# chengruiz/cusrl

Hardware: AMD Instinct MI355X
Metric: env_steps_per_sec (higher is better)
Workload: dtype f32; 1 GPU; synthetic continuous env 4096x obs48 x act12 per GPU, MLP(256,128) actor-critic, rollout_len=24, ppo preset (5 epochs x 4 minibatches, Adam lr 2e-4); envs_per_gpu=4096, parallelism=dp1, rccl_ranks=0, collectives=none (single process), hipgraph=True, fused_env=True, captured_env_steps=24, epoch_graph_updates=432, unjoined_steps_captured=20, autoreset=False

## Files before the change

__graft_entry__.py:

```python

from __future__ import annotations

import os
import subprocess
import sys
from pathlib import Path

ROOT = Path(__file__).resolve().parent
CSRC = ROOT / "cusrl_amd" / "csrc"
LIB = ROOT / "cusrl_amd" / "libcusrl_hip.so"
HIP_SOURCES = ["api.hip", "buffer.hip", "advantage.hip", "ppo_loss.hip", "rollout.hip", "policy_stats.hip", "policy_terms.hip", "mlp_epilogue.hip", "input_layer.hip", "mlp_forward.hip", "gradient.hip", "narrow_linear.hip", "normalization.hip", "recurrent.hip", "aux_hooks.hip", "gru.hip", "comm.hip", "symmetry.hip", "smoothness.hip", "layer_norm.hip", "column_affine.hip", "gate.hip", "attention.hip", "conv.hip", "bijector.hip", "bias_act.hip", "deploy.hip", "environment.hip", "reward_norm.hip", "frame_stack.hip"]
HIPCC_FLAGS = [
    "--offload-arch=gfx950",
    "-O3",
    "-std=c++17",
    "-ffp-contract=off",
    "-fPIC",
    "-shared",
    "-ldl",
]


def _stale(target: Path, sources: list[Path]) -> bool:
    return not target.exists() or any(src.stat().st_mtime > target.stat().st_mtime for src in sources)


def build(force: bool = False) -> None:
    from concurrent.futures import ThreadPoolExecutor

    sources = [CSRC / name for name in HIP_SOURCES]
    headers = [*sorted(CSRC.glob("*.hpp")), ROOT / "include" / "cusrl_hip.h"]
    hipcc = os.environ.get("HIPCC", "/opt/rocm/bin/hipcc")
    objdir = ROOT / "build" / "obj"
    objdir.mkdir(parents=True, exist_ok=True)
    compile_flags = [f for f in HIPCC_FLAGS if f not in ("-shared", "-ldl")]

    def compile_one(src: Path) -> Path:
        obj = objdir / (src.stem + ".o")
        if force or _stale(obj, [src, *headers]):
            subprocess.run([hipcc, *compile_flags, f"-I{ROOT / 'include'}", f"-I{CSRC}", "-c", str(src), "-o", str(obj)], check=True)
        return obj

    with ThreadPoolExecutor(max_workers=min(8, os.cpu_count() or 1)) as pool:
        objects = list(pool.map(compile_one, sources))
    if force or _stale(LIB, objects):
        subprocess.run([hipcc, "--offload-arch=gfx950", "-shared", "-fPIC", "-s", *map(str, objects), "-ldl", "-o", str(LIB)], check=True)
    if str(ROOT) not in sys.path:
        sys.path.insert(0, str(ROOT))
    import oracle

    oracle.build(force=force)
    import cusrl_amd
    from cusrl_amd import _native

    _native.lib()
    assert cusrl_amd.__name__ == "cusrl_amd"


def smoke() -> None:
    if str(ROOT) not in sys.path:
        sys.path.insert(0, str(ROOT))
    import numpy as np
    import torch

    import cusrl_amd as cusrl
    import oracle

    assert torch.cuda.is_available(), "smoke() needs an MI355X"
    cusrl.config.set_device("cuda:0")
    cusrl.set_global_seed(0)
    env = cusrl.testing.SyntheticEnvironment(num_instances=256, observation_dim=48, action_dim=12, device="cuda:0")
    factory = cusrl.preset.PpoAgentFactory(num_steps_per_update=8, sampler_epochs=2, sampler_mini_batches=2)
    trainer = cusrl.Trainer(env, factory, num_iterations=2, verbose=False)
    trainer.run_training_loop()
    buffer = trainer.agent.buffer
    host = {k: buffer[k].cpu().numpy() for k in ("reward", "value", "next_value", "done", "advantage", "return")}
    adv, ret = oracle.gae(host["reward"], host["done"], host["value"], host["next_value"], 0.99, 0.95)
    assert np.array_equal(ret, host["return"]), "return differs from the oracle"
    var, mean = oracle.var_mean(adv)
    np.testing.assert_allclose(oracle.normalize(adv, mean, var), host["advantage"], rtol=1e-5, atol=1e-5)
    torch.cuda.synchronize()
    print("smoke ok: 2 iterations of the ppo preset on cuda:0, GAE/return bit-exact vs oracle")


if __name__ == "__main__":
    build(force="--force" in sys.argv)
    print(f"built {LIB}")
```

cusrl_amd/csrc/narrow_linear.hip:

```cpp
#include <stdlib.h>

#include "common.hpp"

namespace cusrl {

static int head_rows_per_block() {
    const int v = int(option(kOptHeadRows));
    return v >= 8 && v <= 4096 ? v : 96;
}
constexpr int head_batch(int O) { return O > 8 ? 2 : 4; }
constexpr int kHeadBiasPad = 16;

template <int O, bool kReluInput>
__global__ __launch_bounds__(kBlock) void narrow_linear_bwd_kernel(const float *__restrict__ grad_out,
                                                                   const float *__restrict__ input,
                                                                   const float *__restrict__ weight,
                                                                   float *__restrict__ grad_input,
                                                                   float *__restrict__ partials, int64_t rows, int K,
                                                                   int rows_per_block) {
    extern __shared__ float4 red[];
    constexpr int SL = O + 1;
    const int lpr = K / 4;
    const int groups = kBlock / lpr;
    const int col = threadIdx.x % lpr, sub = threadIdx.x / lpr;
// ... 95 lines not shown
            total.x += (a.x + b.x) + (c.x + d.x), total.y += (a.y + b.y) + (c.y + d.y);
            total.z += (a.z + b.z) + (c.z + d.z), total.w += (a.w + b.w) + (c.w + d.w);
        }
        for (; p < P; p += 16) {
            const float4 a = base[p * stride];
            total.x += a.x, total.y += a.y, total.z += a.z, total.w += a.w;
        }
    }
    red[threadIdx.x] = total;
    __syncthreads();
    if (group == 0 && h < H) {
        float4 sum = red[c4];
        for (int g = 1; g < 16; ++g) {
            const float4 v = red[g * 16 + c4];
            sum.x += v.x, sum.y += v.y, sum.z += v.z, sum.w += v.w;
        }
        *reinterpret_cast<float4 *>(out + h) = sum;
    }
}


template <int kLanes>
__global__ __launch_bounds__(kBlock) void narrow_dot_fwd_kernel(const float *__restrict__ input, const float *__restrict__ weight,
                                                                const float *__restrict__ bias, float *__restrict__ output,
                                                                int64_t rows, int K) {
    constexpr int kRowsPerWave = kWave / kLanes, kInFlight = 4;
    const int lane = threadIdx.x & (kWave - 1);
    const int sub = lane % kLanes, rloc = lane / kLanes;
    const int chunks = K / 4;
    const int64_t wave = int64_t(blockIdx.x) * kWavesPerBlock + threadIdx.x / kWave;
    const int64_t row0 = wave * (kRowsPerWave * kInFlight);
    if (row0 >= rows) return;
    const float b = bias ? bias[0] : 0.f;
    float acc[kInFlight] = {0.f, 0.f, 0.f, 0.f};
    for (int c = sub; c < chunks; c += kLanes) {
        const float4 w = reinterpret_cast<const float4 *>(weight)[c];
        float4 x[kInFlight];
#pragma unroll
        for (int k = 0; k < kInFlight; ++k) {
            const int64_t row = min(row0 + int64_t(k) * kRowsPerWave + rloc, rows - 1);
            x[k] = reinterpret_cast<const float4 *>(input)[row * chunks + c];
        }
#pragma unroll
        for (int k = 0; k < kInFlight; ++k)
            acc[k] += (x[k].x * w.x + x[k].y * w.y) + (x[k].z * w.z + x[k].w * w.w);
    }
#pragma unroll
    for (int k = 0; k < kInFlight; ++k) {
        float v = acc[k];
#pragma unroll
        for (int off = kLanes / 2; off > 0; off >>= 1) v += __shfl_xor(v, off, kWave);
        const int64_t row = row0 + int64_t(k) * kRowsPerWave + rloc;
        if (sub == 0 && row < rows) output[row] = v + b;
    }
}

static bool narrow_shape_ok(int64_t K, int64_t O) {
    if (O < 1 || O > 16 || K < 32 || K > 1024 || K % 4) return false;
    const int64_t lpr = K / 4;
    return (lpr & (lpr - 1)) == 0;
}

template <int O, bool kReluInput>
static int launch_narrow_bwd_as(const float *grad_out, const float *input, const float *weight, float *grad_input,
                                float *partials, int64_t rows, int K, int64_t blocks, hipStream_t s) {
    const int lpr = K / 4, groups = kBlock / lpr;
    const size_t lds = size_t(groups) * (O + 1) * lpr * sizeof(float4) + size_t(groups) * kHeadBiasPad * sizeof(float);
    if (lds > 64 * 1024) {
        hipError_t err = hipFuncSetAttribute(reinterpret_cast<const void *>(&narrow_linear_bwd_kernel<O, kReluInput>),
                                             hipFuncAttributeMaxDynamicSharedMemorySize, int(lds));
        if (err != hipSuccess) return int(err);
    }
    hipLaunchKernelGGL((narrow_linear_bwd_kernel<O, kReluInput>), dim3(uint32_t(blocks)), dim3(kBlock), lds, s, grad_out,
                       input, weight, grad_input, partials, rows, K, head_rows_per_block());
    return launch_status();
}

template <int O>
static int launch_narrow_bwd(const float *grad_out, const float *input, const float *weight, float *grad_input,
                             float *partials, int64_t rows, int K, int64_t blocks, bool relu_input, hipStream_t s) {
    return relu_input ? launch_narrow_bwd_as<O, true>(grad_out, input, weight, grad_input, partials, rows, K, blocks, s)
                      : launch_narrow_bwd_as<O, false>(grad_out, input, weight, grad_input, partials, rows, K, blocks, s);
}

}

extern "C" int cusrl_narrow_linear_supported(int64_t in_features, int64_t out_features) {
    return cusrl::narrow_shape_ok(in_features, out_features) ? 1 : 0;
}

extern "C" int64_t cusrl_narrow_linear_num_partials(int64_t rows) {
    return rows <= 0 ? 0 : cusrl::ceil_div(rows, int64_t(cusrl::head_rows_per_block()));
}

extern "C" int cusrl_narrow_linear_bwd(const float *grad_out, const float *input, const float *weight,
                                       float *grad_input, float *partials, float *packed, int64_t rows,
                                       int64_t in_features, int64_t out_features, int relu_input, void *stream) {
    using namespace cusrl;
    if (!grad_out || !input || !weight || !partials || rows <= 0) return CUSRL_E_INVALID;
    if (!narrow_shape_ok(in_features, out_features)) return CUSRL_E_UNSUPPORTED;
    if (out_features % 4 == 0 && !aligned(grad_out, 16)) return CUSRL_E_UNSUPPORTED;
    if (!aligned(input, 16) || !aligned(weight, 16) || !aligned(partials, 16) || (packed && !aligned(packed, 16)) ||
        (grad_input && !aligned(grad_input, 16)))
        return CUSRL_E_UNSUPPORTED;
    hipStream_t s = as_stream(stream);
    const int K = int(in_features);
    const int64_t blocks = ceil_div(rows, int64_t(head_rows_per_block()));
    const bool relu = relu_input != 0;
    int rc = 0;
    switch (out_features) {
#define CUSRL_NARROW_CASE(N) \
    case N: rc = launch_narrow_bwd<N>(grad_out, input, weight, grad_input, partials, rows, K, blocks, relu, s); break;
        CUSRL_NARROW_CASE(1) CUSRL_NARROW_CASE(2) CUSRL_NARROW_CASE(3) CUSRL_NARROW_CASE(4)
        CUSRL_NARROW_CASE(5) CUSRL_NARROW_CASE(6) CUSRL_NARROW_CASE(7) CUSRL_NARROW_CASE(8)
        CUSRL_NARROW_CASE(9) CUSRL_NARROW_CASE(10) CUSRL_NARROW_CASE(11) CUSRL_NARROW_CASE(12)
        CUSRL_NARROW_CASE(13) CUSRL_NARROW_CASE(14) CUSRL_NARROW_CASE(15) CUSRL_NARROW_CASE(16)
#undef CUSRL_NARROW_CASE
        default: return CUSRL_E_UNSUPPORTED;
    }
    if (rc) return rc;
    if (!packed) return 0;
    const int H = (int(out_features) + 1) * K + kHeadBiasPad;
    hipLaunchKernelGGL(narrow_linear_finalize_kernel, dim3(uint32_t(ceil_div(H, 64))), dim3(kBlock), 0, s, partials,
                       blocks, H, packed);
    return launch_status();
}

extern "C" int cusrl_narrow_linear_fwd(const float *input, const float *weight, const float *bias, float *output,
                                       int64_t rows, int64_t in_features, int64_t out_features, void *stream) {
    using namespace cusrl;
    if (!input || !weight || !output || rows <= 0) return CUSRL_E_INVALID;
    if (out_features != 1 || !narrow_shape_ok(in_features, 1)) return CUSRL_E_UNSUPPORTED;
    if (!aligned(input, 16) || !aligned(weight, 16)) return CUSRL_E_UNSUPPORTED;
    const int K = int(in_features), lanes = K / 4 >= kWave ? kWave : K / 4;
    const int64_t waves = ceil_div(rows, int64_t(kWave / lanes) * 4), blocks = ceil_div(waves, int64_t(kWavesPerBlock));
    if (blocks > INT32_MAX) return CUSRL_E_UNSUPPORTED;
    hipStream_t s = as_stream(stream);
    switch (lanes) {
#define CUSRL_DOT_CASE(N)                                                                                              \
    case N:                                                                                                            \
        hipLaunchKernelGGL(narrow_dot_fwd_kernel<N>, dim3(uint32_t(blocks)), dim3(kBlock), 0, s, input, weight, bias,   \
                           output, rows, K);                                                                           \
        break;
        CUSRL_DOT_CASE(8) CUSRL_DOT_CASE(16) CUSRL_DOT_CASE(32) CUSRL_DOT_CASE(64)
#undef CUSRL_DOT_CASE
        default: return CUSRL_E_UNSUPPORTED;
    }
    return launch_status();
}
```

cusrl_amd/nn/module.py:

```python

from __future__ import annotations

from collections.abc import Iterable, Sequence
from contextlib import contextmanager
from dataclasses import dataclass
from typing import Any

import torch
from torch import nn
from torch.nn.functional import linear

from cusrl_amd.utils import switches
from cusrl_amd.utils.nest import iterate_nested

__all__ = ["Linear", "LinearFp32", "fused_inference_layers", "linear_act", "Mlp", "Module", "ModuleFactory", "disable_autocast",
           "double_differentiable", "is_unit_gradient", "register_unit_gradient", "resolve_activation_fn", "saved_gradients"]


def disable_autocast(device_type: str):
    return torch.autocast(device_type=device_type, enabled=False)


_split_grad_sink: dict[int, torch.Tensor] | None = None


_plain_linear_depth = 0
_WIDE_MIN_ROWS = switches.read("WIDE_LINEAR_MIN_ROWS")
_INPUT_LAYER_KERNEL = switches.read("INPUT_LAYER_KERNEL")


_unit_gradients: dict[int, "weakref.ref[torch.Tensor]"] = {}


def register_unit_gradient(ones: torch.Tensor) -> torch.Tensor:
    import weakref

    address = ones.data_ptr()
    _unit_gradients[address] = weakref.ref(ones)
    weakref.finalize(ones, _forget_unit_gradient, address)
    return ones


def _forget_unit_gradient(address: int) -> None:
    ref = _unit_gradients.get(address)
    if ref is not None and ref() is None:
        del _unit_gradients[address]


def is_unit_gradient(grad: torch.Tensor | None) -> bool:
    if grad is None or grad.dim() != 0:
        return False
    ref = _unit_gradients.get(grad.data_ptr())
    return ref is not None and ref() is not None


def saved_gradients(gradients, grad_loss) -> list:
    if is_unit_gradient(grad_loss):
        return list(gradients)
    return [gradient * grad_loss for gradient in gradients]


@contextmanager
def double_differentiable():
    global _plain_linear_depth
    _plain_linear_depth += 1
    try:
        yield
    finally:
        _plain_linear_depth -= 1


@contextmanager
def collect_split_weight_grads():
    global _split_grad_sink
    previous, _split_grad_sink = _split_grad_sink, {}
    try:
        yield _split_grad_sink
    finally:
        _split_grad_sink = previous


def _hand_over(sink, key, gradient):
    from cusrl_amd import ops

    if not isinstance(gradient, ops.DeferredColumns):
        return gradient
    if sink is not None and key is not None and key not in sink:
        sink[key] = gradient
        return None
    return gradient.materialize()


class _WideBatchLinear(torch.autograd.Function):

    @staticmethod
    def forward(ctx, input, weight, bias, splits, relu):
        if relu:
            output = torch._addmm_activation(bias, input, weight.t())
            ctx.save_for_backward(input, weight, output)
            output._cusrl_relu_output = True
        else:
            output = _one_output_linear(input, weight, bias)
            ctx.save_for_backward(input, weight)
        ctx.splits, ctx.relu, ctx.has_bias = splits, relu, bias is not None
        ctx.bias_key = bias.data_ptr() if bias is not None else None
        ctx.narrow = ((not relu) and input.is_contiguous() and weight.is_contiguous() and input.data_ptr() % 16 == 0
                      and _narrow_head(weight))
        ctx.input_is_relu_output = getattr(input, "_cusrl_relu_output", False)
        return output

    @staticmethod
    @torch.autograd.function.once_differentiable
    def backward(ctx, grad_output):
        from cusrl_amd import ops

        if ctx.relu:
            input, weight, output = ctx.saved_tensors
            sink = _split_grad_sink
            premasked = getattr(grad_output, "_cusrl_premasked", None)
            if (_INPUT_LAYER_KERNEL and premasked is None and not ctx.needs_input_grad[0] and ctx.needs_input_grad[1]
                    and ctx.has_bias and ctx.needs_input_grad[2]):
                grad_output = grad_output.contiguous()
                if ops.input_layer_supported(grad_output, output, input, weight):
                    d_weight, d_bias = ops.input_layer_backward(grad_output, output, input)
                    return None, d_weight, d_bias, None, None
            if premasked is not None and premasked[1] == grad_output._version and ctx.has_bias:
                grad_bias = premasked[0]
            else:
                grad_output, grad_bias = ops.relu_backward_bias(
                    grad_output.contiguous(), output, defer=sink is not None and ctx.has_bias and ctx.needs_input_grad[2])
            grad_bias = _hand_over(sink, ctx.bias_key, grad_bias)
        else:
            input, weight = ctx.saved_tensors
            if ctx.narrow and ctx.needs_input_grad[1]:
                fuse_relu = ctx.input_is_relu_output and ctx.needs_input_grad[0]
                sink = _split_grad_sink
                grad_input, grad_weight, grad_bias, masked_colsum = ops.narrow_linear_backward(
                    grad_output.contiguous(), input, weight, need_input_grad=ctx.needs_input_grad[0], relu_input=fuse_relu,
                    defer=sink is not None)
                grad_weight = _hand_over(sink, weight.data_ptr(), grad_weight)
                grad_bias = _hand_over(sink, ctx.bias_key, grad_bias) if ctx.has_bias and ctx.needs_input_grad[2] else None
                if fuse_relu:
                    grad_input._cusrl_premasked = (masked_colsum, grad_input._version)
                return grad_input, grad_weight, (grad_bias if ctx.has_bias else None), None, None
            grad_bias = None
            if ctx.has_bias and ctx.needs_input_grad[2]:
                _, grad_bias = ops.relu_backward_bias(grad_output.contiguous(), None)
        grad_input = grad_weight = None
        if ctx.needs_input_grad[0]:
            grad_input = grad_output @ weight
        if ctx.needs_input_grad[1]:
            rows, splits = input.shape[0], ctx.splits
            if splits > 1:
                gy = grad_output.reshape(splits, rows // splits, -1)
                slabs = torch.bmm(gy.transpose(1, 2), input.reshape(splits, rows // splits, -1))
                sink = _split_grad_sink
                if sink is not None and weight.data_ptr() not in sink:
                    sink[weight.data_ptr()] = slabs
                else:
                    grad_weight = ops.sum_slabs(slabs)
            else:
                grad_weight = grad_output.t() @ input
        return grad_input, grad_weight, grad_bias, None, None


def _one_output_linear(input: torch.Tensor, weight: torch.Tensor, bias: torch.Tensor | None) -> torch.Tensor:
    from cusrl_amd import ops

    if weight.shape[0] == 1 and ops.narrow_linear_forward_supported(input, weight):
        return ops.narrow_linear_forward(input, weight, bias)
    return linear(input, weight, bias)


def _narrow_head(weight: torch.Tensor) -> bool:
    from cusrl_amd import ops

    return (weight.shape[0] <= 16 and weight.data_ptr() % 16 == 0
            and ops.narrow_linear_supported(weight.shape[1], weight.shape[0]))


def _batch_splits(rows: int) -> int:
    if rows < 4096:
        return 1
    splits = 1
    while splits < 32 and rows % (splits * 2) == 0 and rows // (splits * 2) >= 1024:
        splits *= 2
    return splits


def _device_fp32(input: torch.Tensor, weight: torch.Tensor) -> bool:
    return (input.dim() == 2 and input.is_cuda and input.dtype == torch.float32 and weight.dtype == torch.float32
            and not torch.is_autocast_enabled("cuda"))


def linear_act(input: torch.Tensor, weight: torch.Tensor, bias: torch.Tensor | None, relu: bool = False) -> torch.Tensor:
    if _device_fp32(input, weight) and (bias is not None or not relu):
        if (torch.is_grad_enabled() and (weight.requires_grad or input.requires_grad) and input.shape[0] >= _WIDE_MIN_ROWS
                and not _plain_linear_depth):
            return _WideBatchLinear.apply(input, weight, bias, _batch_splits(input.shape[0]), relu)
        if torch.is_grad_enabled() and (weight.requires_grad or input.requires_grad):
            output = linear(input, weight, bias)
            return torch.relu(output) if relu else output
        if relu:
            return torch._addmm_activation(bias, input, weight.t())
        if not torch.is_grad_enabled() or not (weight.requires_grad or input.requires_grad):
            return _one_output_linear(input, weight, bias)
    output = linear(input, weight, bias)
    return torch.relu(output) if relu else output


class Linear(nn.Linear):

    def forward(self, input: torch.Tensor) -> torch.Tensor:
        return linear_act(input, self.weight, self.bias)


class LinearFp32(nn.Linear):

    def forward(self, input: torch.Tensor) -> torch.Tensor:
        if not torch.is_autocast_enabled(input.device.type) and input.dtype == torch.float32:
            return Linear.forward(self, input)
        with disable_autocast(input.device.type):
            return linear(input.float(), self.weight.float(), None if self.bias is None else self.bias.float())


_FUSED_INFERENCE = switches.read("FUSED_INFERENCE")


def fused_inference_layers(backbone, head: nn.Linear, input, memory=None):
    if (not _FUSED_INFERENCE or torch.is_grad_enabled() or memory is not None or not isinstance(backbone, Mlp)
            or not isinstance(head, nn.Linear) or not isinstance(input, torch.Tensor) or not input.is_cuda or input.dim() != 2
            or input.dtype != torch.float32 or torch.is_autocast_enabled("cuda")):
        return None
    stack = backbone.inference_stack()
    if stack is None:
        return None
    from cusrl_amd import ops

    layers = (*stack, head.weight, head.bias)
    return layers if ops.mlp2_forward_supported(input, layers) else None


class ModuleFactory:
    def __call__(self, input_dim: int | None = None, output_dim: int | None = None) -> "Module":
        raise NotImplementedError


class Module(nn.Module):

    Factory = ModuleFactory
    batch_invariant = True

    def __init__(self, input_dim: int | None = None, output_dim: int | None = None, is_recurrent: bool = False,
                 like: "Module | None" = None, intermediate_repr: dict[str, Any] | None = None):
# ... 125 lines not shown
```

cusrl_amd/ops/__init__.py:

```python

from __future__ import annotations

import os
from collections.abc import Sequence

import torch

from cusrl_amd import _native
from cusrl_amd._native import Field, MirrorField, PackedField, check
from cusrl_amd.ops._common import (
    LaunchObserver, _checked, _f32, _flag, _modified_in_place, _observed, _ptr, _raw_stream, _row_bytes, _stream, require_device,
    set_launch_observer,
)
from cusrl_amd.ops.advantage import (
    adv_stats_finalize, col_stats, gae, merge_mean_var, next_value, normalize_, normalize_from_gathered_, normalize_from_partials_,
    packed_mean_var,
)
from cusrl_amd.ops.affine import ColumnAffine, column_affine, column_affine_supported
from cusrl_amd.ops.attention import Rope, Sdpa, rope, rope_supported, sdpa, sdpa_backward, sdpa_supported
from cusrl_amd.ops.band_attention import BandSdpa, band_mask, band_sdpa, band_sdpa_backward, band_sdpa_supported
from cusrl_amd.ops.bias_act import bias_act, bias_act_supported
from cusrl_amd.ops.bijector import BijectorFunction, bijector_supported, sigmoid_bijector, softplus_bijector
from cusrl_amd.ops.auxiliary import (
    accumulate_scalars_, action_smoothness_fwd_bwd, amp_prepare, amp_prepare_supported, amp_style_reward_, amp_style_reward_mean_, bce_pair_fwd_bwd,
    column_mse_fwd_bwd, column_table, masked_col_stats, mse_loss_fwd_bwd, nan_to_num_, normal_nll_bound, normal_nll_fwd_bwd,
    resolve_columns, reward_shaping_, rms_merge_, rms_normalize, rnd_reward_, sumsq_fwd_bwd,
)
from cusrl_amd.ops.buffer import (
    HostCounter, RecordPack, _row_elems, assign_rows, buffer_push, compact_flags, gather_rows, gather_rows_packed, make_push_table,
    push_table, scatter_rows, splice_rows, window_indices,
)
from cusrl_amd.ops.conv import (
    DepthwiseConv2d, depthwise_conv2d, dwconv2d_backward_input, dwconv2d_backward_params, dwconv2d_supported,
)
from cusrl_amd.ops.deploy import deploy_epilogue_, deploy_epilogue_cpu_, deploy_prologue, deploy_prologue_cpu, deploy_supported
from cusrl_amd.ops.environment import (
    CLASSIC_TASKS, ClassicTask, classic_reset, classic_reset_cpu, classic_step, classic_step_cpu,
)
from cusrl_amd.ops.frame_stack import (
    frame_stack_columns, frame_stack_padding, frame_stack_push, frame_stack_push_cpu, frame_stack_reset, frame_stack_reset_cpu,
    frame_stack_supported,
)
from cusrl_amd.ops.gate import GateCombine, Glu, gate_backward, gate_combine, gate_supported, glu, glu_backward, glu_supported
from cusrl_amd.ops.gradient import (
    DeferredColumns, adam_norm_workspace, adam_step, adam_step_normed, adam_step_window, assemble_gradients, clip_grad_norm_,
    grad_sumsq, sum_slabs,
)
from cusrl_amd.ops.graph import graph_census, graph_replace_memsets
from cusrl_amd.ops.layer_norm import AddLayerNorm, add_layer_norm, add_layer_norm_bwd, add_layer_norm_fwd, add_layer_norm_supported
from cusrl_amd.ops.loss import (
    LOSS_DEFER, DeferredLoss, _optional_rows, categorical_policy_stats, categorical_terms_bwd, categorical_terms_fwd, policy_stats,
    policy_terms_bwd, policy_terms_fwd, ppo_loss_accepts_std_vector, ppo_loss_categorical_fwd_bwd, ppo_loss_fwd_bwd,
    value_loss_fwd_bwd,
)
from cusrl_amd.ops.mlp import (
    _HEAD_PAD, input_layer_backward, input_layer_supported, mlp2_forward, mlp2_forward_supported, narrow_linear_backward,
    narrow_linear_forward, narrow_linear_forward_supported, narrow_linear_supported, relu_backward_bias,
)
from cusrl_amd.ops.recurrent import (
    gru_bias_partial_rows, gru_bias_partials_supported, gru_gates_backward, gru_gates_forward, lstm_gates_backward,
    lstm_gates_forward, rnn_cell_backward, rnn_cell_forward,
)
from cusrl_amd.ops.reward import reward_normalize_, reward_normalize_cpu_
from cusrl_amd.ops.rollout import (
    PendingStepEpilogue, categorical_sample_logp, episode_stats, normal_sample_logp, play_epilogue, play_epilogue_workspace,
    step_epilogue, synthetic_env_step,
)
from cusrl_amd.ops.symmetry import (
    _mirror_table, _rows_2d, mirror_mse_fwd_bwd, mirror_rows, mirror_rows_bwd, symmetric_head_bwd, symmetric_head_fwd,
    symmetric_head_sample, symmetric_head_supported, symmetrize_mean_var_,
)
```

cusrl_amd/ops/mlp.py:

```python

from __future__ import annotations

import torch

from cusrl_amd import _native
from cusrl_amd.ops._common import _checked, _f32, _observed, _ptr, _stream
from cusrl_amd.ops.gradient import DeferredColumns


def relu_backward_bias(grad_output: torch.Tensor, output: torch.Tensor | None, defer: bool = False):
    grad_output = _f32(grad_output, "grad_output")
    H = grad_output.shape[-1]
    rows = grad_output.numel() // H
    lib = _native.lib()
    num_partials = max(int(lib.cusrl_colsum_num_partials(rows, H)), 1)
    partials = torch.empty((num_partials, H), dtype=torch.float32, device=grad_output.device)
    chunkable = H % 4 == 0 and H // 4 <= 256 and 256 % (H // 4) == 0
    defer = defer and chunkable and grad_output.data_ptr() % 16 == 0 and (output is None or output.data_ptr() % 16 == 0)
    colsum = None if defer else torch.empty(H, dtype=torch.float32, device=grad_output.device)
    if output is None:
        grad_in, out_ptr, in_ptr = grad_output, None, None
    else:
        output = _f32(output, "output")
        grad_in = torch.empty_like(grad_output)
        out_ptr, in_ptr = output.data_ptr(), grad_in.data_ptr()
    _checked.cusrl_relu_bwd_colsum(grad_output.data_ptr(), out_ptr, in_ptr, partials.data_ptr(), _ptr(colsum), rows, H, _stream())
    return grad_in, (DeferredColumns(partials, num_partials, H, 0, H) if colsum is None else colsum)


def input_layer_supported(grad_output: torch.Tensor, output: torch.Tensor | None, input: torch.Tensor, weight: torch.Tensor) -> bool:
    H, K = weight.shape
    tensors = [grad_output, input] + ([] if output is None else [output])
    return (bool(_native.lib().cusrl_input_layer_supported(K, H)) and input.dim() == 2 and grad_output.shape == (input.shape[0], H)
            and all(t.is_cuda and t.dtype == torch.float32 and t.is_contiguous() and t.data_ptr() % 16 == 0 for t in tensors)
            and (output is None or output.shape == grad_output.shape) and input.shape[0] > 0)


def input_layer_backward(grad_output: torch.Tensor, output: torch.Tensor | None, input: torch.Tensor) -> tuple[torch.Tensor, torch.Tensor]:
    grad_output, input = _f32(grad_output, "grad_output"), _f32(input, "input")
    rows, K = input.shape
    H = grad_output.shape[-1]
    lib = _native.lib()
    dev = input.device
    width = H * K + H
    partials = torch.empty((int(lib.cusrl_input_layer_row_blocks(rows, H)), width), dtype=torch.float32, device=dev)
    grads = torch.empty(width, dtype=torch.float32, device=dev)
    _observed("cusrl_input_layer_bwd", grad_output.data_ptr(), _ptr(None if output is None else _f32(output, "output")),
            input.data_ptr(), rows, K, H, partials.data_ptr(), grads.data_ptr(),
            nbytes=lambda: rows * 4 * ((2 if output is not None else 1) * H + K) + (partials.numel() * 2 + width) * 4)
    return grads[: H * K].view(H, K), grads[H * K :]


_HEAD_PAD = 16


def narrow_linear_supported(in_features: int, out_features: int) -> bool:
    return bool(_native.lib().cusrl_narrow_linear_supported(in_features, out_features))


def narrow_linear_forward_supported(input: torch.Tensor, weight: torch.Tensor) -> bool:
    return (weight.dim() == 2 and weight.shape[0] == 1 and input.dim() == 2 and input.is_cuda and input.dtype == torch.float32
            and weight.dtype == torch.float32 and input.is_contiguous() and weight.is_contiguous() and input.shape[0] > 0
            and input.data_ptr() % 16 == 0 and weight.data_ptr() % 16 == 0 and narrow_linear_supported(weight.shape[1], 1))


def narrow_linear_forward(input: torch.Tensor, weight: torch.Tensor, bias: torch.Tensor | None) -> torch.Tensor:
    input, weight = _f32(input, "input"), _f32(weight, "weight")
    rows, K = input.shape
    out = torch.empty((rows, 1), dtype=torch.float32, device=input.device)
    _checked.cusrl_narrow_linear_fwd(input.data_ptr(), weight.data_ptr(), _ptr(None if bias is None else _f32(bias, "bias")),
            out.data_ptr(), rows, K, 1, _stream())
    return out


def mlp2_forward_supported(input: torch.Tensor, layers) -> bool:
    w1, b1, w2, b2, w3, b3 = layers
    tensors = [input, w1, b1, w2, b2, w3] + ([b3] if b3 is not None else [])
    if input.dim() != 2 or input.shape[0] == 0 or any(
            (not t.is_cuda) or t.dtype != torch.float32 or (not t.is_contiguous()) or t.data_ptr() % 16 for t in tensors):
        return False
    if w1.dim() != 2 or w2.dim() != 2 or w3.dim() != 2 or w1.shape[1] != input.shape[1] or w2.shape[1] != w1.shape[0] \
            or w3.shape[1] != w2.shape[0] or b1.numel() != w1.shape[0] or b2.numel() != w2.shape[0] \
            or (b3 is not None and b3.numel() != w3.shape[0]):
        return False
    return bool(_native.lib().cusrl_mlp2_forward_supported(w1.shape[1], w1.shape[0], w2.shape[0], w3.shape[0]))


def mlp2_forward(input: torch.Tensor, layers, std: torch.Tensor | None = None, eps: torch.Tensor | None = None,
                 repeat_std: bool = True):
    w1, b1, w2, b2, w3, b3 = layers
    input = _f32(input, "input")
    rows, K = input.shape
    out_features = w3.shape[0]
    out = torch.empty((rows, out_features), dtype=torch.float32, device=input.device)
    sampling = eps is not None
    action = logp = repeated = None
    if sampling:
        std, eps = _f32(std, "std"), _f32(eps, "eps")
        if std.numel() != out_features or eps.shape != out.shape:
            raise ValueError("mlp2_forward: one std per output and one eps per output element are required")
        action = torch.empty_like(out)
        logp = torch.empty((rows, 1), dtype=torch.float32, device=input.device)
        repeated = torch.empty_like(out) if repeat_std else None
    _observed(
        "cusrl_mlp2_forward", input.data_ptr(), rows, K, w1.data_ptr(), b1.data_ptr(), w1.shape[0], w2.data_ptr(),
        b2.data_ptr(), w2.shape[0], w3.data_ptr(), _ptr(b3), out_features, out.data_ptr(),
        _ptr(std) if sampling else None, _ptr(eps), _ptr(action), _ptr(logp), _ptr(repeated),
        nbytes=lambda: rows * 4 * (K + out_features * (4 if sampling else 1)) + 4 * (w1.numel() + w2.numel() + w3.numel()),
    )
    if sampling:
        return action, logp, out, repeated
    return out


def narrow_linear_backward(grad_output: torch.Tensor, input: torch.Tensor, weight: torch.Tensor,
                           need_input_grad: bool = True, relu_input: bool = False, defer: bool = False):
    grad_output, input, weight = _f32(grad_output, "grad_output"), _f32(input, "input"), _f32(weight, "weight")
    O, K = weight.shape
    rows = input.shape[0]
    lib = _native.lib()
    dev = input.device
    grad_input = torch.empty_like(input) if need_input_grad else None
    width = (O + 1) * K + _HEAD_PAD
    num_partials = int(lib.cusrl_narrow_linear_num_partials(rows))
    partials = torch.empty((num_partials, width), dtype=torch.float32, device=dev)
    packed = None if defer else torch.empty(width, dtype=torch.float32, device=dev)
    _checked.cusrl_narrow_linear_bwd(grad_output.data_ptr(), input.data_ptr(), weight.data_ptr(), _ptr(grad_input),
            partials.data_ptr(), _ptr(packed), rows, K, O, int(relu_input), _stream())
    if defer:
        window = lambda column, numel: DeferredColumns(partials, num_partials, width, column, numel)
        return grad_input, window(0, O * K), window((O + 1) * K, O), (window(O * K, K) if relu_input else None)
    colsum = packed[O * K : (O + 1) * K] if relu_input else None
    return grad_input, packed[: O * K].view(O, K), packed[(O + 1) * K : (O + 1) * K + O], colsum
```

include/cusrl_hip.h:

```cpp
#ifndef CUSRL_HIP_H
#define CUSRL_HIP_H

#include <stdint.h>

#ifdef __cplusplus
extern "C" {
#endif

#define CUSRL_ABI_VERSION 7
#define CUSRL_MAX_FIELDS 24
#define CUSRL_MAX_PACKED 16
#define CUSRL_MAX_RECORD_BYTES 1024
#define CUSRL_MAX_MIRROR_FIELDS 24
#define CUSRL_MAX_SYMMETRIZE_CHANNELS 4096
#define CUSRL_MAX_SYMMETRIC_HEAD_ACTIONS 64

#define CUSRL_E_INVALID (-1)
#define CUSRL_E_TOO_MANY (-2)
#define CUSRL_E_UNSUPPORTED (-3)
#define CUSRL_E_COMM (-4)

typedef struct {
    const void *src;
    void *dst;
// ... 98 lines not shown
                        const int64_t *lengths, int64_t t, int64_t B, int64_t H, void *stream);
int cusrl_gru_gates_bwd_bias(float *gi, float *gh, const float *b_hh, const float *h_prev, const float *d_out, float *dh,
                             const int64_t *lengths, int64_t t, int64_t B, int64_t H, float *bias_partials, void *stream);
int64_t cusrl_gru_bias_partial_rows(int64_t B);
int cusrl_gru_bias_supported(int64_t H, const float *gi, const float *gh, const float *b_hh, const float *h_prev,
                             const float *d_out, const float *dh, const float *bias_partials);

int cusrl_lstm_gates_fwd(float *gi, const float *gh, const float *b_hh, float *h, float *c, float *out, float *c_saved,
                         const int64_t *lengths, int64_t t, int64_t B, int64_t H, void *stream);
int cusrl_lstm_gates_bwd(float *pre, const float *c_prev, const float *c_next, const float *d_out, float *dh, float *dc,
                         const int64_t *lengths, int64_t t, int64_t B, int64_t H, void *stream);

int cusrl_rnn_cell_fwd(const float *gi, const float *gh, const float *b_hh, float *h, float *out, const int64_t *lengths,
                       int64_t t, int64_t B, int64_t H, int relu, void *stream);
int cusrl_rnn_cell_bwd(float *d_pre, const float *out, const float *d_out, float *dh, const int64_t *lengths, int64_t t,
                       int64_t B, int64_t H, int relu, void *stream);

int cusrl_normal_sample_logp(const float *mean, const float *std, const float *eps, float *action, float *logp,
                             int64_t B, int64_t A, int64_t std_rows, float *std_out, const float *mean_bias,
                             float *mean_out, void *stream);

int cusrl_categorical_sample_logp(const float *logits, const float *noise, float *action, float *logp, int64_t B,
                                  int64_t A, void *stream);

int cusrl_episode_stats(const float *reward, const uint8_t *done, float *episode_rew, float *episode_len,
                        float *ring_rew, float *ring_len, uint64_t *num_episodes, double *step_reward_sum,
                        int64_t N, int64_t D, int64_t R, int parity, void *stream);

int cusrl_step_epilogue(const float *reward, const uint8_t *terminated, const uint8_t *truncated, uint8_t *done_out,
                        float *episode_rew, float *episode_len, float *ring_rew, float *ring_len, uint64_t *num_episodes,
                        double *step_reward_sum, int64_t *indices_out, int32_t *count_out, int64_t N, int64_t D, int64_t R,
                        int parity, void *stream);
int64_t cusrl_step_epilogue_max_envs(void);
int cusrl_step_epilogue_push(const float *reward, const uint8_t *terminated, const uint8_t *truncated, uint8_t *done_out,
                             float *episode_rew, float *episode_len, float *ring_rew, float *ring_len, uint64_t *num_episodes,
                             double *step_reward_sum, int64_t *indices_out, int32_t *count_out, int64_t N, int64_t D, int64_t R,
                             int parity, const cusrl_field_t *fields, int n_fields, int done_field, int64_t cursor,
                             void *stream);

int cusrl_play_epilogue(const float *reward, const uint8_t *terminated, const uint8_t *truncated, uint8_t *done_out,
                        float *episode_rew, float *episode_len, float *ring_rew, float *ring_len, uint64_t *num_episodes,
                        double *step_reward_sum, int64_t *indices_out, int32_t *count_out, int64_t N, int64_t D, int64_t R,
                        int parity, int64_t *episode_count, int64_t target_episodes, int32_t *unfinished_out,
                        uint32_t *workspace, void *stream);
int64_t cusrl_play_epilogue_workspace_words(void);

int cusrl_policy_stats(const float *old_mean, const float *old_std, const float *new_mean, const float *new_std,
                       const float *action, const float *old_logp, const float *advantage, int64_t B, int64_t A,
                       int64_t D, double *partials, float *out, void *stream);
int64_t cusrl_policy_stats_num_partials(int64_t B);
int cusrl_categorical_policy_stats(const float *old_logits, const float *new_logits, const float *action,
                                   const float *old_logp, const float *advantage, int64_t B, int64_t A, int64_t D,
                                   double *partials, float *out, void *stream);

int cusrl_policy_terms_fwd(const float *mean, const float *std, int64_t std_rows, const float *action,
                           const float *old_logp, int64_t B, int64_t A, float *logp_out, float *entropy_out,
                           float *logp_ratio_out, float *ratio_out, void *stream);
int cusrl_policy_terms_bwd(const float *mean, const float *std, int64_t std_rows, const float *action, const float *ratio,
                           const float *g_logp, const float *g_entropy, const float *g_logp_ratio, const float *g_ratio,
                           int64_t B, int64_t A, float *d_mean, float *d_std, float *d_std_partials, void *stream);
int64_t cusrl_policy_terms_std_partial_rows(int64_t B);
int cusrl_categorical_terms_fwd(const float *logits, const float *action, const float *old_logp, int64_t B, int64_t A,
                                float *logp_out, float *entropy_out, float *logp_ratio_out, float *ratio_out, void *stream);
int cusrl_categorical_terms_bwd(const float *logits, const float *action, const float *ratio, const float *g_logp,
                                const float *g_entropy, const float *g_logp_ratio, const float *g_ratio, int64_t B,
                                int64_t A, float *d_logits, void *stream);

int cusrl_relu_bwd_colsum(const float *grad, const float *output, float *grad_in, float *partials, float *colsum,
                          int64_t rows, int64_t H, void *stream);
int64_t cusrl_colsum_num_partials(int64_t rows, int64_t H);

int cusrl_input_layer_bwd(const float *grad_out, const float *output, const float *input, int64_t rows, int64_t in_features,
                          int64_t out_features, float *partials, float *grads, void *stream);
int cusrl_input_layer_supported(int64_t in_features, int64_t out_features);
int64_t cusrl_input_layer_row_blocks(int64_t rows, int64_t out_features);

int cusrl_narrow_linear_bwd(const float *grad_out, const float *input, const float *weight, float *grad_input,
                            float *partials, float *packed, int64_t rows, int64_t in_features, int64_t out_features,
                            int relu_input, void *stream);
int64_t cusrl_narrow_linear_num_partials(int64_t rows);
int cusrl_narrow_linear_supported(int64_t in_features, int64_t out_features);
int cusrl_narrow_linear_fwd(const float *input, const float *weight, const float *bias, float *output, int64_t rows,
                            int64_t in_features, int64_t out_features, void *stream);

int cusrl_mlp2_forward(const float *input, int64_t rows, int64_t in_features, const float *w1, const float *b1, int64_t hidden1,
                       const float *w2, const float *b2, int64_t hidden2, const float *w3, const float *b3, int64_t out_features,
                       float *output, const float *std, const float *eps, float *action, float *logp, float *std_out,
                       void *stream);
int cusrl_mlp2_forward_supported(int64_t in_features, int64_t hidden1, int64_t hidden2, int64_t out_features);

int cusrl_clip_grad_norm(float *grad, int64_t n, float max_norm, double *partials, float *norm_out, void *stream);
int64_t cusrl_clip_grad_norm_num_partials(int64_t n);

typedef struct {
    const void *src;
    int64_t offset;
    int64_t numel;
    int64_t splits;
    int64_t row_stride;
} cusrl_grad_piece_t;
int cusrl_assemble_gradients(const cusrl_grad_piece_t *pieces, int64_t num_pieces, float *flat, double *sumsq_partials,
                             void *stream);
int64_t cusrl_assemble_gradients_blocks(const cusrl_grad_piece_t *pieces, int64_t num_pieces);

int cusrl_grad_sumsq(const float *grad, int64_t n, double *partials, void *stream);

int cusrl_adam_step(float *param, const float *grad, float *exp_avg, float *exp_avg_sq, float *step, const float *lr,
                    int64_t n, double beta1, double beta2, double eps, double weight_decay, int decoupled_weight_decay,
                    int maximize, const double *clip_partials, int64_t num_clip_partials, float max_norm,
                    float *norm_out, float *norm_accumulator, uint32_t *ticket, void *stream);

int cusrl_adam_step_window(float *param, const float *grad, float *exp_avg, float *exp_avg_sq, float *step, const float *lr,
                           int64_t n, double beta1, double beta2, double eps, double weight_decay, int decoupled_weight_decay,
                           int maximize, const double *clip_partials_a, int64_t num_a, const double *clip_partials_b,
                           int64_t num_b, float max_norm, float *norm_out, float *norm_accumulator, float *step_mirror,
                           uint32_t *ticket, void *stream);

int cusrl_adam_step_normed(float *param, const float *grad, float *exp_avg, float *exp_avg_sq, float *step, const float *lr,
                           int64_t n, double beta1, double beta2, double eps, double weight_decay, int decoupled_weight_decay,
                           int maximize, const float *norm_grad, int64_t norm_n, void *workspace, float max_norm, float *norm_out,
                           float *norm_accumulator, float *step_mirror, uint32_t *ticket, void *stream);
int64_t cusrl_adam_step_normed_workspace_bytes(void);

int cusrl_masked_col_stats(const float *x, const uint8_t *mask, int64_t rows, int64_t C, double *partials,
                           float *batch_mean, float *batch_var, double *batch_count, void *stream);
int64_t cusrl_masked_stats_num_partials(int64_t rows, int64_t C);

int cusrl_rms_merge(float *mean, float *var, float *std, double *count, const float *batch_mean,
                    const float *batch_var, const double *batch_count, float eps, double max_count, int64_t C,
                    void *stream);

int cusrl_rms_normalize(const float *x, const float *mean, const float *std, float clamp, float *out, int64_t rows,
                        int64_t C, void *stream);

int cusrl_sequence_count(const uint8_t *done, int64_t L, int64_t N, int32_t *env_prefix, int32_t *block_totals,
                         int32_t *num_sequences, void *stream);
int64_t cusrl_sequence_blocks(int64_t N);
int cusrl_sequence_layout(const uint8_t *done, int64_t L, int64_t N, const int32_t *env_prefix,
                          const int32_t *block_totals, int64_t Ns, int64_t *dest, int64_t *first_seq, uint8_t *mask,
                          int64_t *seq_lengths, int64_t *last_seq, void *stream);
int cusrl_gather_memory(const void *memory, const int64_t *last_seq, const uint8_t *done_last, void *out, int64_t N,
                        int64_t row_bytes, void *stream);

int cusrl_rnd_reward(const float *target, const float *prediction, float *reward, float *bonus_out, float scale,
                     int64_t rows, int64_t K, void *stream);
int cusrl_amp_style_reward(const float *logit, float *reward, float *bonus_out, float scale, int64_t rows, void *stream);
int cusrl_amp_style_reward_mean(const float *logit, float *reward, float *bonus_out, float scale, int64_t rows,
                                float *mean_out, void *stream);

int cusrl_amp_prepare(const float *state, const float *next_state, int64_t state_pitch, const int32_t *columns, int64_t K,
                      const float *agent_raw, const float *dataset, const int64_t *indices, const float *expert_raw,
                      int64_t N, int64_t C, float *mean, float *var, float *std, double *count, float eps,
                      double max_count, float clamp, float *agent_out, float *expert_out, double *workspace, void *stream);
int64_t cusrl_amp_prepare_max_elements(void);
int64_t cusrl_amp_prepare_workspace(int64_t N, int64_t C);

int cusrl_synthetic_env_step(uint64_t seed, uint64_t *counter, int64_t N, int64_t obs_dim, int64_t reward_dim,
                             float p_terminate, float p_truncate, float *next_observation, float *reward,
                             uint8_t *terminated, uint8_t *truncated, float *reset_rows, void *stream);

int cusrl_accumulate_scalars(const float *const *values, int n, float *accumulator, void *stream);

int cusrl_reward_shaping(float *reward, float scale, float shift, float lower, float upper, int has_lower, int has_upper,
                         int64_t n, void *stream);

int cusrl_nan_to_num2(float *a, int64_t na, float *b, int64_t nb, float nan, float posinf, float neginf, void *stream);
// ... 191 lines not shown
```

Measured before the change: 20.37 million env-steps/s.

## Add MFMA kernels for input-layer linear+ReLU and narrow multi-output heads

Adds two MFMA-based HIP kernels. The first is a persistent, double-buffered input-layer linear+ReLU forward that keeps weights in registers and stages output tiles through LDS. The second is a narrow-head forward for 2-16 outputs. The module routes the bottom ReLU layer (when the input needs no grad) and multi-output heads to these kernels instead of rocBLAS addmm/linear, to cut per-call GEMM overhead on skinny shapes. The new paths only cover a limited set of shapes and fall back to the old calls otherwise.

```diff
diff --git a/__graft_entry__.py b/__graft_entry__.py
--- a/__graft_entry__.py
+++ b/__graft_entry__.py
@@ -9,7 +9,7 @@
 ROOT = Path(__file__).resolve().parent
 CSRC = ROOT / "cusrl_amd" / "csrc"
 LIB = ROOT / "cusrl_amd" / "libcusrl_hip.so"
-HIP_SOURCES = ["api.hip", "buffer.hip", "advantage.hip", "ppo_loss.hip", "rollout.hip", "policy_stats.hip", "policy_terms.hip", "mlp_epilogue.hip", "input_layer.hip", "mlp_forward.hip", "gradient.hip", "narrow_linear.hip", "normalization.hip", "recurrent.hip", "aux_hooks.hip", "gru.hip", "comm.hip", "symmetry.hip", "smoothness.hip", "layer_norm.hip", "column_affine.hip", "gate.hip", "attention.hip", "conv.hip", "bijector.hip", "bias_act.hip", "deploy.hip", "environment.hip", "reward_norm.hip", "frame_stack.hip"]
+HIP_SOURCES = ["api.hip", "buffer.hip", "advantage.hip", "ppo_loss.hip", "rollout.hip", "policy_stats.hip", "policy_terms.hip", "mlp_epilogue.hip", "input_layer.hip", "mlp_forward.hip", "gradient.hip", "narrow_linear.hip", "thin_linear.hip", "normalization.hip", "recurrent.hip", "aux_hooks.hip", "gru.hip", "comm.hip", "symmetry.hip", "smoothness.hip", "layer_norm.hip", "column_affine.hip", "gate.hip", "attention.hip", "conv.hip", "bijector.hip", "bias_act.hip", "deploy.hip", "environment.hip", "reward_norm.hip", "frame_stack.hip"]
 HIPCC_FLAGS = [
     "--offload-arch=gfx950",
     "-O3",
diff --git a/cusrl_amd/csrc/narrow_linear.hip b/cusrl_amd/csrc/narrow_linear.hip
--- a/cusrl_amd/csrc/narrow_linear.hip
+++ b/cusrl_amd/csrc/narrow_linear.hip
@@ -201,6 +201,9 @@
     return relu_input ? launch_narrow_bwd_as<O, true>(grad_out, input, weight, grad_input, partials, rows, K, blocks, s)
                       : launch_narrow_bwd_as<O, false>(grad_out, input, weight, grad_input, partials, rows, K, blocks, s);
 }
+
+int launch_narrow_rows_fwd(const float *input, const float *weight, const float *bias, float *output, int64_t rows, int64_t K,
+                           int64_t A, hipStream_t s);
 
 }
 
@@ -249,6 +252,8 @@
                                        int64_t rows, int64_t in_features, int64_t out_features, void *stream) {
     using namespace cusrl;
     if (!input || !weight || !output || rows <= 0) return CUSRL_E_INVALID;
+    if (out_features > 1)
+        return launch_narrow_rows_fwd(input, weight, bias, output, rows, in_features, out_features, as_stream(stream));
     if (out_features != 1 || !narrow_shape_ok(in_features, 1)) return CUSRL_E_UNSUPPORTED;
     if (!aligned(input, 16) || !aligned(weight, 16)) return CUSRL_E_UNSUPPORTED;
     const int K = int(in_features), lanes = K / 4 >= kWave ? kWave : K / 4;
diff --git a/cusrl_amd/csrc/thin_linear.hip b/cusrl_amd/csrc/thin_linear.hip
--- /dev/null
+++ b/cusrl_amd/csrc/thin_linear.hip
@@ -0,0 +1,210 @@
+#include "common.hpp"
+
+namespace cusrl {
+
+typedef float thin_f32x4 __attribute__((ext_vector_type(4)));
+
+constexpr int kThinRows = 16;
+
+__device__ __forceinline__ thin_f32x4 thin_relu4(thin_f32x4 v) {
+    v[0] = v[0] <= 0.f ? 0.f : v[0], v[1] = v[1] <= 0.f ? 0.f : v[1], v[2] = v[2] <= 0.f ? 0.f : v[2], v[3] = v[3] <= 0.f ? 0.f : v[3];
+    return v;
+}
+
+template <int T, int KB>
+__global__ __launch_bounds__(kBlock) void input_linear_relu_fwd_kernel(const float *__restrict__ x, const float *__restrict__ w,
+                                                                       const float *__restrict__ b, float *__restrict__ y,
+                                                                       int64_t rows, int K) {
+    constexpr int H = 64 * T, kPitch = H + 4, kChunks = H / 4;
+    __shared__ __attribute__((aligned(16))) float stage[2][kThinRows][kPitch];
+    const int lane = threadIdx.x & (kWave - 1), wave = threadIdx.x / kWave;
+    const int i = lane & 15, kk = lane >> 4;
+    const float4 zero4 = make_float4(0.f, 0.f, 0.f, 0.f);
+
+    float4 a[T][KB];
+    thin_f32x4 c[T];
+#pragma unroll
+    for (int t1 = 0; t1 < T; ++t1) {
+        const int n = 16 * (T * wave + t1);
+#pragma unroll
+        for (int t = 0; t < KB; ++t) {
+            const int k = 16 * t + 4 * kk;
+            const float4 v = *reinterpret_cast<const float4 *>(w + int64_t(n + i) * K + (k < K ? k : 0));
+            a[t1][t] = k < K ? v : zero4;
+        }
+        const float4 bias = *reinterpret_cast<const float4 *>(b + n + 4 * kk);
+        c[t1] = thin_f32x4{bias.x, bias.y, bias.z, bias.w};
+    }
+    const int64_t tiles = (rows + kThinRows - 1) / kThinRows;
+    float4 ahead[KB];
+    auto request = [&](int64_t tile) {
+        const int64_t row = min(tile * kThinRows + i, rows - 1);
+#pragma unroll
+        for (int t = 0; t < KB; ++t) {
+            const int k = 16 * t + 4 * kk;
+            ahead[t] = *reinterpret_cast<const float4 *>(x + row * K + (k < K ? k : 0));
+        }
+    };
+    request(min(int64_t(blockIdx.x), tiles - 1));
+    int buffer = 0;
+    for (int64_t tile = blockIdx.x; tile < tiles; tile += gridDim.x) {
+        const int64_t row0 = tile * kThinRows;
+        float4 xb[KB];
+#pragma unroll
+        for (int t = 0; t < KB; ++t) xb[t] = 16 * t + 4 * kk < K ? ahead[t] : zero4;
+        request(min(tile + gridDim.x, tiles - 1));
+        thin_f32x4 acc[T];
+#pragma unroll
+        for (int t1 = 0; t1 < T; ++t1) acc[t1] = c[t1];
+#pragma unroll
+        for (int t = 0; t < KB; ++t) {
+            const float bv[4] = {xb[t].x, xb[t].y, xb[t].z, xb[t].w};
+#pragma unroll
+            for (int j = 0; j < 4; ++j)
+#pragma unroll
+                for (int t1 = 0; t1 < T; ++t1) {
+                    const float av = j == 0 ? a[t1][t].x : j == 1 ? a[t1][t].y : j == 2 ? a[t1][t].z : a[t1][t].w;
+                    acc[t1] = __builtin_amdgcn_mfma_f32_16x16x4f32(av, bv[j], acc[t1], 0, 0, 0);
+                }
+        }
+#pragma unroll
+        for (int t1 = 0; t1 < T; ++t1) {
+            const thin_f32x4 r = thin_relu4(acc[t1]);
+            *reinterpret_cast<float4 *>(&stage[buffer][i][16 * (T * wave + t1) + 4 * kk]) = make_float4(r[0], r[1], r[2], r[3]);
+        }
+        __syncthreads();
+#pragma unroll
+        for (int r = 0; r < T; ++r) {
+            const int f = int(threadIdx.x) + kBlock * r;
+            const int row = f / kChunks, chunk = f % kChunks;
+            if (row0 + row < rows)
+                *reinterpret_cast<float4 *>(y + (row0 + row) * H + 4 * chunk) = *reinterpret_cast<const float4 *>(&stage[buffer][row][4 * chunk]);
+        }
+        buffer ^= 1;
+    }
+}
+
+template <int T>
+static int launch_input_linear(const float *x, const float *w, const float *b, float *y, int64_t rows, int K, dim3 grid, hipStream_t s) {
+    switch ((K + 15) / 16) {
+        case 1: hipLaunchKernelGGL((input_linear_relu_fwd_kernel<T, 1>), grid, dim3(kBlock), 0, s, x, w, b, y, rows, K); break;
+        case 2: hipLaunchKernelGGL((input_linear_relu_fwd_kernel<T, 2>), grid, dim3(kBlock), 0, s, x, w, b, y, rows, K); break;
+        case 3: hipLaunchKernelGGL((input_linear_relu_fwd_kernel<T, 3>), grid, dim3(kBlock), 0, s, x, w, b, y, rows, K); break;
+        case 4: hipLaunchKernelGGL((input_linear_relu_fwd_kernel<T, 4>), grid, dim3(kBlock), 0, s, x, w, b, y, rows, K); break;
+        default: return CUSRL_E_UNSUPPORTED;
+    }
+    return launch_status();
+}
+
+template <int KB>
+__global__ __launch_bounds__(kBlock) void narrow_rows_fwd_kernel(const float *__restrict__ x, const float *__restrict__ w,
+                                                                 const float *__restrict__ b, float *__restrict__ y, int64_t rows,
+                                                                 int A) {
+    constexpr int K = 16 * KB;
+    const int lane = threadIdx.x & (kWave - 1);
+    const int i = lane & 15, kk = lane >> 4;
+    const float4 zero4 = make_float4(0.f, 0.f, 0.f, 0.f);
+    float4 a[KB];
+#pragma unroll
+    for (int t = 0; t < KB; ++t) {
+        const float4 v = *reinterpret_cast<const float4 *>(w + int64_t(i < A ? i : 0) * K + 16 * t + 4 * kk);
+        a[t] = i < A ? v : zero4;
+    }
+    thin_f32x4 c = {0.f, 0.f, 0.f, 0.f};
+    if (b) {
+#pragma unroll
+        for (int reg = 0; reg < 4; ++reg) c[reg] = 4 * kk + reg < A ? b[4 * kk + reg] : 0.f;
+    }
+    const int64_t tiles = (rows + kThinRows - 1) / kThinRows;
+    const int64_t waves = int64_t(gridDim.x) * kWavesPerBlock;
+    const bool wide_store = A % 4 == 0;
+    for (int64_t tile = int64_t(blockIdx.x) * kWavesPerBlock + threadIdx.x / kWave; tile < tiles; tile += waves) {
+        const int64_t row = tile * kThinRows + i;
+        const float *from = x + min(row, rows - 1) * K + 4 * kk;
+        float4 xb[KB];
+#pragma unroll
+        for (int t = 0; t < KB; ++t) xb[t] = *reinterpret_cast<const float4 *>(from + 16 * t);
+        thin_f32x4 even = c, odd = {0.f, 0.f, 0.f, 0.f};
+#pragma unroll
+        for (int t = 0; t < KB; t += 2) {
+            const float a0[4] = {a[t].x, a[t].y, a[t].z, a[t].w}, b0[4] = {xb[t].x, xb[t].y, xb[t].z, xb[t].w};
+            const float a1[4] = {a[t + 1].x, a[t + 1].y, a[t + 1].z, a[t + 1].w}, b1[4] = {xb[t + 1].x, xb[t + 1].y, xb[t + 1].z, xb[t + 1].w};
+#pragma unroll
+            for (int j = 0; j < 4; ++j) {
+                even = __builtin_amdgcn_mfma_f32_16x16x4f32(a0[j], b0[j], even, 0, 0, 0);
+                odd = __builtin_amdgcn_mfma_f32_16x16x4f32(a1[j], b1[j], odd, 0, 0, 0);
+            }
+        }
+        const int a_first = 4 * kk;
+        if (row < rows && a_first < A) {
+            float *to = y + row * A + a_first;
+            if (wide_store) {
+                *reinterpret_cast<float4 *>(to) = make_float4(even[0] + odd[0], even[1] + odd[1], even[2] + odd[2], even[3] + odd[3]);
+            } else {
+#pragma unroll
+                for (int reg = 0; reg < 4; ++reg)
+                    if (a_first + reg < A) to[reg] = even[reg] + odd[reg];
+            }
+        }
+    }
+}
+
+static int compute_units() {
+    static int cus = 0;
+    if (cus == 0) {
+        int device = 0, count = 0;
+        if (hipGetDevice(&device) != hipSuccess || hipDeviceGetAttribute(&count, hipDeviceAttributeMultiprocessorCount, device) != hipSuccess || count <= 0)
+            count = 256;
+        cus = count;
+    }
+    return cus;
+}
+
+static bool narrow_rows_shape_ok(int64_t K, int64_t A) { return A >= 2 && A <= 16 && (K == 64 || K == 128 || K == 256); }
+
+int launch_narrow_rows_fwd(const float *input, const float *weight, const float *bias, float *output, int64_t rows, int64_t K,
+                           int64_t A, hipStream_t s) {
+    if (!narrow_rows_shape_ok(K, A)) return CUSRL_E_UNSUPPORTED;
+    if (!aligned(input, 16) || !aligned(weight, 16) || (A % 4 == 0 && !aligned(output, 16))) return CUSRL_E_UNSUPPORTED;
+    const int64_t tiles = ceil_div(rows, kThinRows);
+    const int64_t blocks = min(ceil_div(tiles, int64_t(kWavesPerBlock)), int64_t(compute_units()) * 8);
+    const dim3 grid{uint32_t(blocks)};
+    switch (K) {
+        case 64: hipLaunchKernelGGL(narrow_rows_fwd_kernel<4>, grid, dim3(kBlock), 0, s, input, weight, bias, output, rows, int(A)); break;
+        case 128: hipLaunchKernelGGL(narrow_rows_fwd_kernel<8>, grid, dim3(kBlock), 0, s, input, weight, bias, output, rows, int(A)); break;
+        default: hipLaunchKernelGGL(narrow_rows_fwd_kernel<16>, grid, dim3(kBlock), 0, s, input, weight, bias, output, rows, int(A)); break;
+    }
+    return launch_status();
+}
+
+}
+
+using namespace cusrl;
+
+extern "C" int cusrl_input_linear_relu_supported(int64_t in_features, int64_t out_features) {
+    return in_features >= 4 && in_features <= 64 && in_features % 4 == 0 && out_features >= 64 && out_features <= 256 &&
+           out_features % 64 == 0;
+}
+
+extern "C" int cusrl_narrow_linear_fwd_supported(int64_t in_features, int64_t out_features) {
+    return out_features == 1 ? cusrl_narrow_linear_supported(in_features, 1) : narrow_rows_shape_ok(in_features, out_features) ? 1 : 0;
+}
+
+extern "C" int cusrl_input_linear_relu_fwd(const float *input, const float *weight, const float *bias, float *output, int64_t rows,
+                                           int64_t in_features, int64_t out_features, int64_t workgroups, void *stream) {
+    if (!input || !weight || !bias || !output || rows <= 0 || workgroups < 0 || workgroups > (1 << 20)) return CUSRL_E_INVALID;
+    if (!cusrl_input_linear_relu_supported(in_features, out_features)) return CUSRL_E_UNSUPPORTED;
+    if (!aligned(input, 16) || !aligned(weight, 16) || !aligned(bias, 16) || !aligned(output, 16)) return CUSRL_E_UNSUPPORTED;
+    const int64_t tiles = ceil_div(rows, kThinRows);
+    constexpr int kThinGroupsPerCu = 2;
+    const int64_t wanted = workgroups > 0 ? workgroups : int64_t(compute_units()) * kThinGroupsPerCu;
+    const dim3 grid{uint32_t(tiles < wanted ? tiles : wanted)};
+    hipStream_t s = as_stream(stream);
+    const int K = int(in_features);
+    switch (out_features / 64) {
+        case 1: return launch_input_linear<1>(input, weight, bias, output, rows, K, grid, s);
+        case 2: return launch_input_linear<2>(input, weight, bias, output, rows, K, grid, s);
+        case 3: return launch_input_linear<3>(input, weight, bias, output, rows, K, grid, s);
+        default: return launch_input_linear<4>(input, weight, bias, output, rows, K, grid, s);
+    }
+}
diff --git a/cusrl_amd/nn/module.py b/cusrl_amd/nn/module.py
--- a/cusrl_amd/nn/module.py
+++ b/cusrl_amd/nn/module.py
@@ -27,6 +27,7 @@
 _plain_linear_depth = 0
 _WIDE_MIN_ROWS = switches.read("WIDE_LINEAR_MIN_ROWS")
 _INPUT_LAYER_KERNEL = switches.read("INPUT_LAYER_KERNEL")
+THIN_LINEAR_FORWARD = True
 
 
 _unit_gradients: dict[int, "weakref.ref[torch.Tensor]"] = {}
@@ -96,11 +97,11 @@
     @staticmethod
     def forward(ctx, input, weight, bias, splits, relu):
         if relu:
-            output = torch._addmm_activation(bias, input, weight.t())
+            output = _bottom_layer_relu(input, weight, bias, ctx.needs_input_grad[0])
             ctx.save_for_backward(input, weight, output)
             output._cusrl_relu_output = True
         else:
-            output = _one_output_linear(input, weight, bias)
+            output = _narrow_output_linear(input, weight, bias)
             ctx.save_for_backward(input, weight)
         ctx.splits, ctx.relu, ctx.has_bias = splits, relu, bias is not None
         ctx.bias_key = bias.data_ptr() if bias is not None else None
@@ -164,12 +165,28 @@
         return grad_input, grad_weight, grad_bias, None, None
 
 
+def _bottom_layer_relu(input: torch.Tensor, weight: torch.Tensor, bias: torch.Tensor, input_needs_grad: bool) -> torch.Tensor:
+    from cusrl_amd import ops
+
+    if THIN_LINEAR_FORWARD and not input_needs_grad and ops.input_linear_relu_supported(input, weight, bias):
+        return ops.input_linear_relu(input, weight, bias)
+    return torch._addmm_activation(bias, input, weight.t())
+
+
 def _one_output_linear(input: torch.Tensor, weight: torch.Tensor, bias: torch.Tensor | None) -> torch.Tensor:
     from cusrl_amd import ops
 
     if weight.shape[0] == 1 and ops.narrow_linear_forward_supported(input, weight):
         return ops.narrow_linear_forward(input, weight, bias)
     return linear(input, weight, bias)
+
+
+def _narrow_output_linear(input: torch.Tensor, weight: torch.Tensor, bias: torch.Tensor | None) -> torch.Tensor:
+    from cusrl_amd import ops
+
+    if THIN_LINEAR_FORWARD and weight.shape[0] >= 2 and ops.narrow_head_forward_supported(input, weight, bias):
+        return ops.narrow_head_forward(input, weight, bias)
+    return _one_output_linear(input, weight, bias)
 
 
 def _narrow_head(weight: torch.Tensor) -> bool:
diff --git a/cusrl_amd/ops/__init__.py b/cusrl_amd/ops/__init__.py
--- a/cusrl_amd/ops/__init__.py
+++ b/cusrl_amd/ops/__init__.py
@@ -54,8 +54,9 @@
     value_loss_fwd_bwd,
 )
 from cusrl_amd.ops.mlp import (
-    _HEAD_PAD, input_layer_backward, input_layer_supported, mlp2_forward, mlp2_forward_supported, narrow_linear_backward,
-    narrow_linear_forward, narrow_linear_forward_supported, narrow_linear_supported, relu_backward_bias,
+    _HEAD_PAD, input_layer_backward, input_layer_supported, input_linear_relu, input_linear_relu_supported, mlp2_forward,
+    mlp2_forward_supported, narrow_head_forward, narrow_head_forward_supported, narrow_linear_backward, narrow_linear_forward,
+    narrow_linear_forward_supported, narrow_linear_supported, relu_backward_bias,
 )
 from cusrl_amd.ops.recurrent import (
     gru_bias_partial_rows, gru_bias_partials_supported, gru_gates_backward, gru_gates_forward, lstm_gates_backward,
diff --git a/cusrl_amd/ops/mlp.py b/cusrl_amd/ops/mlp.py
--- a/cusrl_amd/ops/mlp.py
+++ b/cusrl_amd/ops/mlp.py
@@ -73,6 +73,45 @@
     return out
 
 
+def _plain_f32(*tensors: torch.Tensor) -> bool:
+    return all(t.is_cuda and t.dtype == torch.float32 and t.is_contiguous() and t.data_ptr() % 16 == 0 for t in tensors)
+
+
+def narrow_head_forward_supported(input: torch.Tensor, weight: torch.Tensor, bias: torch.Tensor | None) -> bool:
+    return (weight.dim() == 2 and weight.shape[0] >= 2 and input.dim() == 2 and input.shape[0] > 0 and input.shape[1] == weight.shape[1]
+            and _plain_f32(input, weight) and (bias is None or (_plain_f32(bias) and bias.numel() == weight.shape[0]))
+            and bool(_native.lib().cusrl_narrow_linear_fwd_supported(weight.shape[1], weight.shape[0])))
+
+
+def narrow_head_forward(input: torch.Tensor, weight: torch.Tensor, bias: torch.Tensor | None) -> torch.Tensor:
+    input, weight = _f32(input, "input"), _f32(weight, "weight")
+    rows, K = input.shape
+    out = torch.empty((rows, weight.shape[0]), dtype=torch.float32, device=input.device)
+    _checked.cusrl_narrow_linear_fwd(input.data_ptr(), weight.data_ptr(), _ptr(None if bias is None else _f32(bias, "bias")),
+            out.data_ptr(), rows, K, weight.shape[0], _stream())
+    return out
+
+
+def input_linear_relu_supported(input: torch.Tensor, weight: torch.Tensor, bias: torch.Tensor | None) -> bool:
+    return (bias is not None and weight.dim() == 2 and input.dim() == 2 and input.shape[0] > 0 and input.shape[1] == weight.shape[1]
+            and bias.numel() == weight.shape[0] and _plain_f32(input, weight, bias)
+            and bool(_native.lib().cusrl_input_linear_relu_supported(weight.shape[1], weight.shape[0])))
+
+
+def input_linear_relu(input: torch.Tensor, weight: torch.Tensor, bias: torch.Tensor, out: torch.Tensor | None = None,
+                      workgroups: int = 0) -> torch.Tensor:
+    input, weight, bias = _f32(input, "input"), _f32(weight, "weight"), _f32(bias, "bias")
+    rows, K = input.shape
+    H = weight.shape[0]
+    if out is None:
+        out = torch.empty((rows, H), dtype=torch.float32, device=input.device)
+    elif out.shape != (rows, H) or out.dtype != torch.float32 or not out.is_contiguous():
+        raise ValueError("input_linear_relu: out must be a contiguous float32 [rows, out_features] tensor")
+    _checked.cusrl_input_linear_relu_fwd(input.data_ptr(), weight.data_ptr(), bias.data_ptr(), out.data_ptr(), rows, K, H,
+            int(workgroups), _stream())
+    return out
+
+
 def mlp2_forward_supported(input: torch.Tensor, layers) -> bool:
     w1, b1, w2, b2, w3, b3 = layers
     tensors = [input, w1, b1, w2, b2, w3] + ([b3] if b3 is not None else [])
diff --git a/include/cusrl_hip.h b/include/cusrl_hip.h
--- a/include/cusrl_hip.h
+++ b/include/cusrl_hip.h
@@ -204,6 +204,11 @@
 int cusrl_narrow_linear_supported(int64_t in_features, int64_t out_features);
 int cusrl_narrow_linear_fwd(const float *input, const float *weight, const float *bias, float *output, int64_t rows,
                             int64_t in_features, int64_t out_features, void *stream);
+int cusrl_narrow_linear_fwd_supported(int64_t in_features, int64_t out_features);
+
+int cusrl_input_linear_relu_fwd(const float *input, const float *weight, const float *bias, float *output, int64_t rows,
+                                int64_t in_features, int64_t out_features, int64_t workgroups, void *stream);
+int cusrl_input_linear_relu_supported(int64_t in_features, int64_t out_features);
 
 int cusrl_mlp2_forward(const float *input, int64_t rows, int64_t in_features, const float *w1, const float *b1, int64_t hidden1,
                        const float *w2, const float *b2, int64_t hidden2, const float *w3, const float *b3, int64_t out_features,
```

Result: faster. 20.97 million env-steps/s (median of 6 runs) (+3.0%).
